# MeryylleA/Lunaris-Orion

Measured on AMD Instinct MI355X. Metric: 128x128 sprites/sec, VAE training step (train_hybrid.py _process_batch), latent_dim=512, higher is better.
Workload: dtype f16; 1 GPU; VAE-only training step (fwd+MSE/KL+bwd+clip+AdamW), per-GPU batch 64, latent_dim 512, teacher scalar 0 (--reward_scale 0 --quality_weight 0; the full hybrid step of BASELINE config 3 is the config3_full_hybrid object of a --full run at N=1), gradient_accumulation_steps 1, fp16 MFMA operands / fp32 accumulate, fp32 master weights; global_batch=64, latent_dim=512, parallelism=single, linear_weight_gradients=factored (never materialised)

## Files before the change

lunaris_orion_amd/csrc/lo_edge.hip:

```cpp
#include "lo_common.h"
#include <stdlib.h>

#define FC_W 128
#define FC_OW 64
#define FC_CO 64

__device__ __forceinline__ void fc_stage_rows(const float* __restrict__ x, float (*xs)[3][FC_W + 2], int n, int oy, int tid) {
  for (int i = tid; i < 3 * 3 * (FC_W + 2); i += 256) {
    int col = i % (FC_W + 2);
    int r = (i / (FC_W + 2)) % 3;
    int ci = i / (3 * (FC_W + 2));
    int iy = 2 * oy - 1 + r, ix = col - 1;
    float v = 0.f;
    if ((unsigned)iy < 128u && (unsigned)ix < 128u) v = x[(((size_t)n * 3 + ci) * 128 + iy) * 128 + ix];
    xs[ci][r][col] = v;
  }
}

template <int ROWS>
__global__ __launch_bounds__(256) void lo_first_conv_fwd_mfma_kernel(const float* __restrict__ x, const float* __restrict__ w,
                                                                     const float* __restrict__ bias, f16* __restrict__ v,
                                                                     float* __restrict__ gn_partial) {
  constexpr int NR = 2 * ROWS + 1, RP = FC_W + 2;
  __shared__ float xs[3][NR][RP];
  __shared__ float ws[FC_CO * 27];
  __shared__ __attribute__((aligned(16))) unsigned char so[FC_OW * 144];
  __shared__ float red[4][8][2];
  const int tid = threadIdx.x, lane = tid & 63, wave = tid >> 6, m = lane & 15, g = lane >> 4;
  const int oy0 = blockIdx.x * ROWS, n = blockIdx.y;
  for (int i = tid; i < 3 * NR * RP; i += 256) {
    const int col = i % RP, r = (i / RP) % NR, ci = i / (RP * NR);
    const int iy = 2 * oy0 - 1 + r, ix = col - 1;
    float val = 0.f;
    if ((unsigned)iy < 128u && (unsigned)ix < 128u) val = x[(((size_t)n * 3 + ci) * 128 + iy) * 128 + ix];
    xs[ci][r][col] = val;
  }
  for (int i = tid; i < FC_CO * 27; i += 256) ws[i] = w[i];
  __syncthreads();
  f16x8 wh[4], wl[4];
#pragma unroll
  for (int mf = 0; mf < 4; ++mf)
#pragma unroll
    for (int j = 0; j < 8; ++j) {
      const int k = 8 * g + j;
      const float wv = k < 27 ? ws[(16 * mf + m) * 27 + k] : 0.f;
      const f16 hi = (f16)wv;
      wh[mf][j] = hi;
      wl[mf][j] = (f16)(wv - (float)hi);
    }
  int koff[8];
#pragma unroll
  for (int j = 0; j < 8; ++j) {
    const int k = 8 * g + j, kk = k < 27 ? k : 0;
    const int ci = kk / 9, r = (kk % 9) / 3, sx = kk % 3;
    koff[j] = (ci * NR + r) * RP + sx;
  }
  f32x4 bv[4];
#pragma unroll
  for (int mf = 0; mf < 4; ++mf) bv[mf] = *reinterpret_cast<const f32x4*>(bias + 16 * mf + 4 * g);
  const float* xbase = &xs[0][0][0];
  const int px = 16 * wave + m;
#pragma unroll 1
  for (int rr = 0; rr < ROWS; ++rr) {
    f16x8 xh, xl;
#pragma unroll
    for (int j = 0; j < 8; ++j) {
      float xv = xbase[koff[j] + 2 * rr * RP + 2 * px];
      if (8 * g + j >= 27) xv = 0.f;
      const f16 hi = (f16)xv;
      xh[j] = hi;
      xl[j] = (f16)(xv - (float)hi);
    }
    float gs[4], gq[4];
#pragma unroll
    for (int mf = 0; mf < 4; ++mf) {
      f32x4 acc = bv[mf];
      acc = __builtin_amdgcn_mfma_f32_16x16x32_f16(wh[mf], xh, acc, 0, 0, 0);
      acc = __builtin_amdgcn_mfma_f32_16x16x32_f16(wl[mf], xh, acc, 0, 0, 0);
      acc = __builtin_amdgcn_mfma_f32_16x16x32_f16(wh[mf], xl, acc, 0, 0, 0);
      const f16x4 h = {(f16)acc[0], (f16)acc[1], (f16)acc[2], (f16)acc[3]};
      *reinterpret_cast<f16x4*>(so + px * 144 + (16 * mf + 4 * g) * 2) = h;
      float s_ = 0.f, q_ = 0.f;
#pragma unroll
      for (int j = 0; j < 4; ++j) { const float a = (float)h[j]; s_ += a; q_ += a * a; }
      gs[mf] = s_; gq[mf] = q_;
    }
#pragma unroll
    for (int mf = 0; mf < 4; ++mf) {
#pragma unroll
      for (int o = 1; o < 32; o <<= 1) { gs[mf] += __shfl_xor(gs[mf], o, 64); gq[mf] += __shfl_xor(gq[mf], o, 64); }
    }
    if (m == 0 && (g & 1) == 0) {
#pragma unroll
      for (int mf = 0; mf < 4; ++mf) { red[wave][2 * mf + (g >> 1)][0] = gs[mf]; red[wave][2 * mf + (g >> 1)][1] = gq[mf]; }
    }
    __syncthreads();
    const int oy = oy0 + rr;
    {
      f16* dst = v + (((size_t)n * 64 + oy) * 64) * FC_CO;
#pragma unroll
      for (int i = 0; i < 2; ++i) {
        const int c = tid + 256 * i, p = c >> 3, ch = c & 7;
        *reinterpret_cast<u32x4*>(dst + p * FC_CO + ch * 8) = *reinterpret_cast<const u32x4*>(so + p * 144 + ch * 16);
      }
    }
    if (tid < 16) {
      const int grp = tid >> 1, which = tid & 1;
      gn_partial[(((size_t)n * 64 + oy) * 8 + grp) * 2 + which] = red[0][grp][which] + red[1][grp][which] + red[2][grp][which] + red[3][grp][which];
    }
    __syncthreads();
  }
}

template <int ROWS>
__global__ __launch_bounds__(256) void lo_first_conv_wgrad_mfma_kernel(const float* __restrict__ x, const f16* __restrict__ dv,
                                                                       float* __restrict__ partial) {
  __shared__ float xs[3][3][FC_W + 2];
  __shared__ __attribute__((aligned(16))) f16 ds[64][FC_CO];
  __shared__ __attribute__((aligned(16))) f16 xt[2][32][64 + 8];
  const int tid = threadIdx.x, n = blockIdx.y, rb = blockIdx.x;
  const int lane = tid & 63, wave = tid >> 6, i16 = lane & 15, q = lane >> 4;
  f32x4 acc[4];
#pragma unroll
  for (int t = 0; t < 4; ++t) acc[t] = (f32x4){0.f, 0.f, 0.f, 0.f};
  constexpr int XN = (3 * 3 * (FC_W + 2) + 255) / 256;
  f16x8 pd[2];
  float px[XN];
  auto prefetch = [&](int oy) __attribute__((always_inline)) {
    const f16* src = dv + (((size_t)n * 64 + oy) * 64) * FC_CO;
#pragma unroll
    for (int j = 0; j < 2; ++j) pd[j] = reinterpret_cast<const f16x8*>(src)[tid + 256 * j];
#pragma unroll
    for (int j = 0; j < XN; ++j) {
      const int i = tid + 256 * j;
      const int col = i % (FC_W + 2), r = (i / (FC_W + 2)) % 3, ci = i / (3 * (FC_W + 2));
      const int iy = 2 * oy - 1 + r, ix = col - 1;
      float v = 0.f;
      if (i < 3 * 3 * (FC_W + 2) && (unsigned)iy < 128u && (unsigned)ix < 128u) v = x[(((size_t)n * 3 + ci) * 128 + iy) * 128 + ix];
      px[j] = v;
    }
  };
  prefetch(rb * ROWS);
  for (int oy = rb * ROWS; oy < rb * ROWS + ROWS; ++oy) {
    __syncthreads();
#pragma unroll
    for (int j = 0; j < 2; ++j) reinterpret_cast<f16x8*>(&ds[0][0])[tid + 256 * j] = pd[j];
#pragma unroll
    for (int j = 0; j < XN; ++j) {
      const int i = tid + 256 * j;
      if (i < 3 * 3 * (FC_W + 2)) (&xs[0][0][0])[i] = px[j];
    }
    if (oy + 1 < rb * ROWS + ROWS) prefetch(oy + 1);
    __syncthreads();
    for (int i = tid; i < 32 * 64; i += 256) {
      const int k = i >> 6, p = i & 63;
      float v = 0.f;
      if (k < 27) {
        const int ci = k / 9, r = (k % 9) / 3, sx = k % 3;
        v = xs[ci][r][2 * p + sx];
      }
      const f16 hi = (f16)v;
      xt[0][k][p] = hi;
      xt[1][k][p] = (f16)(v - (float)hi);
    }
    __syncthreads();
#pragma unroll
    for (int ks = 0; ks < 2; ++ks) {
      const unsigned char* dbase = reinterpret_cast<const unsigned char*>(&ds[0][0]) + (size_t)(32 * ks + 4 * q + (i16 >> 2)) * 128 + wave * 32 + (i16 & 3) * 8;
      h16x4 a_lo = __builtin_amdgcn_ds_read_tr16_b64_v4f16((h16x4 __attribute__((address_space(3)))*)(dbase));
      h16x4 a_hi = __builtin_amdgcn_ds_read_tr16_b64_v4f16((h16x4 __attribute__((address_space(3)))*)(dbase + 16 * 128));
      const f16x8 af = {(f16)a_lo[0], (f16)a_lo[1], (f16)a_lo[2], (f16)a_lo[3], (f16)a_hi[0], (f16)a_hi[1], (f16)a_hi[2], (f16)a_hi[3]};
#pragma unroll
      for (int t = 0; t < 4; ++t) {
        const f16* xr = &xt[t >> 1][16 * (t & 1) + i16][32 * ks + 4 * q];
// ... 32 lines not shown
    for (; k < nrow; k += 16) t += partial[(size_t)k * stride + j];
  }
  red[r][c] = t;
  __syncthreads();
  if (r == 0 && j < ncol) {
    float tot = 0.f;
#pragma unroll
    for (int q = 0; q < 16; ++q) tot += red[q][c];
    out[j] = tot * scale;
  }
}

#define LC_T 16
#define LC_TP (LC_T + 2)
#define LC_CI 32
#define LC_PITCH 80

__device__ __forceinline__ void lc_stage_a4_wide(const f16* __restrict__ a4, unsigned char* tile, int n, int ty, int tx, int tid) {
  constexpr int NCH = LC_TP * LC_TP * 4, NIT = (NCH + 255) / 256;
  u32x4 v[NIT];
#pragma unroll
  for (int k = 0; k < NIT; ++k) {
    const int i = tid + k * 256;
    const int ch = i & 3, p = i >> 2;
    const int y = p / LC_TP, xx = p % LC_TP;
    const int iy = ty * LC_T - 1 + y, ix = tx * LC_T - 1 + xx;
    v[k] = (u32x4){0u, 0u, 0u, 0u};
    if (i < NCH && (unsigned)iy < 128u && (unsigned)ix < 128u)
      v[k] = *reinterpret_cast<const u32x4*>(a4 + (((size_t)n * 128 + iy) * 128 + ix) * LC_CI + ch * 8);
  }
#pragma unroll
  for (int k = 0; k < NIT; ++k) {
    const int i = tid + k * 256;
    if (i < NCH) *reinterpret_cast<u32x4*>(tile + (i >> 2) * LC_PITCH + (i & 3) * 16) = v[k];
  }
}

__device__ __forceinline__ float lc_tanh(float x) { return 1.f - 2.f * __frcp_rn(__expf(2.f * x) + 1.f); }

__global__ __launch_bounds__(256) void lo_final_conv_fwd_mfma_kernel(const f16* __restrict__ a4, const float* __restrict__ w,
                                                                     const float* __restrict__ bias, const float* __restrict__ target,
                                                                     float* __restrict__ recon, float* __restrict__ mse_partial) {
  __shared__ __attribute__((aligned(16))) unsigned char tile[LC_TP * LC_TP * LC_PITCH];
  __shared__ __attribute__((aligned(16))) f16 wf[9 * 4 * 6 * 8];
  __shared__ float red[4];
  const int tid = threadIdx.x, tx = blockIdx.x, ty = blockIdx.y, n = blockIdx.z;
  const int lane = tid & 63, wave = tid >> 6, m = lane & 15, g = lane >> 4;
  lc_stage_a4_wide(a4, tile, n, ty, tx, tid);
  for (int i = tid; i < 3 * LC_CI * 9; i += 256) {
    const int t = i % 9, ci = (i / 9) % LC_CI, co = i / (9 * LC_CI);
    const float wv = w[i];
    const f16 hi = (f16)wv;
    const int slot = ((t * 4 + (ci >> 3)) * 6 + co) * 8 + (ci & 7);
    wf[slot] = hi;
    wf[slot + 24] = (f16)(wv - (float)hi);
  }
  const float bv = m < 3 ? bias[m] : 0.f;
  __syncthreads();
  f16x8 wb[9];
#pragma unroll
  for (int t = 0; t < 9; ++t) {
    wb[t] = (f16x8){0, 0, 0, 0, 0, 0, 0, 0};
    if (m < 6) wb[t] = *reinterpret_cast<const f16x8*>(&wf[((t * 4 + g) * 6 + m) * 8]);
  }
  float sq = 0.f;
#pragma unroll
  for (int rr = 0; rr < 4; ++rr) {
    const int py = wave * 4 + rr;
    f32x4 acc = {0.f, 0.f, 0.f, 0.f};
#pragma unroll
    for (int t = 0; t < 9; ++t) {
      const int r = t / 3, sx = t % 3;
      const f16x8 af = *reinterpret_cast<const f16x8*>(tile + ((py + r) * LC_TP + m + sx) * LC_PITCH + g * 16);
      acc = __builtin_amdgcn_mfma_f32_16x16x32_f16(af, wb[t], acc, 0, 0, 0);
    }
    f32x4 lo;
#pragma unroll
    for (int j = 0; j < 4; ++j) lo[j] = __shfl_down(acc[j], 3, 64);
    if (m < 3) {
      const int oy = ty * LC_T + py, ox = tx * LC_T + 4 * g;
      const size_t o = (((size_t)n * 3 + m) * 128 + oy) * 128 + ox;
      f32x4 rv;
#pragma unroll
      for (int j = 0; j < 4; ++j) rv[j] = lc_tanh(acc[j] + lo[j] + bv);
      *reinterpret_cast<f32x4*>(recon + o) = rv;
      if (mse_partial) {
        const f32x4 tv = *reinterpret_cast<const f32x4*>(target + o);
#pragma unroll
        for (int j = 0; j < 4; ++j) { const float d = rv[j] - tv[j]; sq += d * d; }
      }
    }
  }
  if (mse_partial) {
    const float e = lo_wave_sum(sq);
    if (lane == 0) red[wave] = e;
    __syncthreads();
    if (tid == 0) mse_partial[((size_t)n * gridDim.y + ty) * gridDim.x + tx] = red[0] + red[1] + red[2] + red[3];
  }
}

struct LcBwdArgs {
  const f16* a4;
  const float* w;
  const float* recon;
  const float* target;
  const float* drecon;
  const float* coef;
  float gscale;
  f16* da4;
  float* partial;
};

__device__ __attribute__((aligned(256))) unsigned int lo_zero_page_e[64];
static_assert(sizeof(lo_zero_page_e) >= 1 * 16, "lc_dma_a4: 16 B per lane, all lanes at offset 0 of the zero page");
static_assert(sizeof(lo_zero_page_e) >= 64 * 4, "lc_dma_rt: 64 lanes x 4 B, lane-linear in the zero page");
#define LC_PATCH_BYTES (21 * 1024)
__device__ __forceinline__ void lc_dma_a4(const f16* __restrict__ a4, unsigned int lds_base, int n, int ty, int tx, int wave, int lane) {
  const unsigned char* zpage = reinterpret_cast<const unsigned char*>(lo_zero_page_e);
#pragma unroll
  for (int i = 0; i < 6; ++i) {
    const int k = wave + 4 * i;
    if (k >= 21) break;
    const int q = k * 64 + lane, p = q >> 2, slot = q & 3;
    const int y = p / LC_TP, xx = p - y * LC_TP;
    const int iy = ty * LC_T - 1 + y, ix = tx * LC_T - 1 + xx;
    const void* src = zpage;
    if (p < LC_TP * LC_TP && (unsigned)iy < 128u && (unsigned)ix < 128u) src = a4 + (((size_t)n * 128 + iy) * 128 + ix) * LC_CI + slot * 8;
    lo_dma16(src, __builtin_amdgcn_readfirstlane(lds_base + k * 1024));
  }
}
__device__ __forceinline__ void lo_dma4(const void* gptr, unsigned int lds_off) {
  asm volatile("s_mov_b32 m0, %1\n\ts_nop 0\n\tglobal_load_lds_dword %0, off" ::"v"(gptr), "s"(lds_off) : "memory");
}
__device__ __forceinline__ void lc_dma_rt(const float* __restrict__ recon, const float* __restrict__ gsrc, unsigned int lds_base, int n,
                                          int ty, int tx, int wave, int lane) {
  const unsigned char* zpage = reinterpret_cast<const unsigned char*>(lo_zero_page_e);
#pragma unroll
  for (int jb = 0; jb < 2; ++jb) {
    const int j = wave + 4 * jb;
    if (j * 64 >= LC_TP * LC_TP) break;
    const int p = j * 64 + lane;
    const int y = p / LC_TP, xx = p - y * LC_TP;
    const int iy = ty * LC_T - 1 + y, ix = tx * LC_T - 1 + xx;
    const bool in = p < LC_TP * LC_TP && (unsigned)iy < 128u && (unsigned)ix < 128u;
    const size_t o = ((size_t)n * 3 * 128 + iy) * 128 + ix;
#pragma unroll
    for (int c = 0; c < 3; ++c) {
      lo_dma4(in ? (const void*)(recon + o + c * 16384) : (const void*)(zpage + lane * 4), __builtin_amdgcn_readfirstlane(lds_base + ((0 * 3 + c) * 384 + j * 64) * 4));
// ... 149 lines not shown
  LoProfScope _p("lo_first_conv_wgrad(+sum)", 2.0 * B * 4096 * 64 * 27, (double)B * (3 * 16384 * 4 + 4096 * 64 * 2), st);
  hipLaunchKernelGGL((lo_first_conv_wgrad_mfma_kernel<4>), dim3(16, B), dim3(256), 0, st, x, dv, partial);
  LO_LAUNCH_CHECK("first_conv_wgrad");
  hipLaunchKernelGGL(lo_colsum_kernel, dim3((1728 + 15) / 16), dim3(256), 0, st, partial, dw, B * 16, 1728, 1728, scale);
  LO_LAUNCH_CHECK("first_conv_wgrad_sum");
  return LO_OK;
}
int lo_colsum(const float* partial, float* out, int nrow, int ncol, int stride, float scale, hipStream_t st) {
  hipLaunchKernelGGL(lo_colsum_kernel, dim3((ncol + 15) / 16), dim3(256), 0, st, partial, out, nrow, ncol, stride, scale);
  LO_LAUNCH_CHECK("colsum");
  return LO_OK;
}
int lo_final_conv_fwd(const f16* a4, const float* w, const float* bias, const float* target, float* recon,
                      float* mse_partial, int B, hipStream_t st) {
  LoProfScope _p("lo_final_conv_fwd", 2.0 * B * 16384 * 3 * 288, (double)B * 16384 * (32 * 2 + 3 * 4 * 2), st);
  hipLaunchKernelGGL(lo_final_conv_fwd_mfma_kernel, dim3(8, 8, B), dim3(256), 0, st, a4, w, bias, target, recon, mse_partial);
  LO_LAUNCH_CHECK("final_conv_fwd");
  return LO_OK;
}
int lo_final_conv_bwd(const f16* a4, const float* w, const float* recon, const float* target, const float* drecon,
                      const float* coef, float gscale, f16* da4, float* partial, float* dw, float* db, int B, float scale,
                      hipStream_t st, hipStream_t sum_st, hipEvent_t sum_after) {
  LcBwdArgs a{a4, w, recon, target, drecon, coef, gscale, da4, partial};
  LoProfScope _p("lo_final_conv_bwd(+sums)", 4.0 * B * 16384 * 3 * 288, (double)B * 16384 * (32 * 2 * 2 + 3 * 4 * 2), st);
  constexpr int rows = 8;
  LO_LAUNCH_STOP(lo_final_conv_bwd_kernel<8>, dim3(rows, B), dim3(256), 0, st, a);
  LO_LAUNCH_CHECK("final_conv_bwd");
  if (sum_st && sum_after) { LO_HIP(hipStreamWaitEvent(sum_st, sum_after, 0)); st = sum_st; }
  hipLaunchKernelGGL(lo_colsum_kernel, dim3((864 + 15) / 16), dim3(256), 0, st, partial, dw, B * rows, 864, 867, scale);
  LO_LAUNCH_CHECK("final_conv_dw");
  hipLaunchKernelGGL(lo_colsum_kernel, dim3(1), dim3(256), 0, st, partial + 864, db, B * rows, 3, 867, scale);
// ... 4 lines not shown
```

lunaris_orion_amd/csrc/lo_norm.h:

```cpp
#pragma once
#include "lo_common.h"

int lo_gn_nchunk(int HW, int C);
bool lo_gn_bwd_local_applies(int HW, int C);

struct LoGnLayer { const f16* v; const float* stats; const float* gamma; const float* beta; int B, HW, C; };

struct LoGnFwd {
  const float* partial = nullptr; int MT = 0;
  const float* slab = nullptr; int nsplit = 0; const float* bias = nullptr;
  const f16* other = nullptr;
  int mode = 0;
  f16* y = nullptr;
  uint8_t* y8 = nullptr;
};
int lo_gn_forward(const LoGnLayer& l, const LoGnFwd& op, hipStream_t st);

struct LoGnBwd {
  const f16* dy = nullptr;
  const float* slab = nullptr; int nsplit = 0; const f16* add_src = nullptr; f16* dy_out = nullptr;
  const f16* other = nullptr;
  int mode = 0;
  f16* ds = nullptr;
  f16* dv = nullptr;
// ... 6 lines not shown
enum LoGnBwdForm {
  LO_GNB_SLAB_LOCAL,
  LO_GNB_APPLY_ONLY,
  LO_GNB_LOCAL,
  LO_GNB_TWO_PASS
};
struct LoGnUse { bool slab = false; int rows_in_P1 = 0; bool allow_local = false; };
static inline LoGnUse lo_gn_use(const LoGnBwd& op) { return {op.slab != nullptr, op.rows_in_P1, op.allow_local}; }
struct LoGnChoice { LoGnBwdForm form; LoGnRows rows; };
LoGnChoice lo_gn_bwd_choose(int HW, int C, const LoGnUse& use);
int lo_gn_backward(const LoGnLayer& l, const LoGnBwd& op, hipStream_t st, LoGnRows* rows = nullptr);
int lo_gn_bwd(const LoGnLayer& l, const LoGnBwd& op, float* dgamma, float* dbeta, float* dbias, float scale, hipStream_t st);

struct LoGnFinJob { const float* P1; const float* P2; float* dgamma; float* dbeta; float* dbias; int nblk1, nblk2, C, block0; };
#define LO_GN_FIN_MAX 16
struct LoGnFinJobs { LoGnFinJob j[LO_GN_FIN_MAX]; int n; };
int lo_gn_finalize_all(const LoGnFinJobs& jobs, float scale, hipStream_t st);

int lo_nhwc_to_nchw_f16(const f16* src, f16* dst, int B, int HW, int C, hipStream_t st);
int lo_nchw_to_nhwc_f16(const f16* src, f16* dst, int B, int HW, int C, hipStream_t st, uint8_t* dst8 = nullptr);
int lo_nhwc_f16_to_nchw_f32(const f16* src, float* dst, int B, int HW, int C, float scale, hipStream_t st);
int lo_nchw_f32_to_nhwc_f16(const float* src, f16* dst, int B, int HW, int C, float scale, hipStream_t st);
```

lunaris_orion_amd/csrc/lo_norm.hip:

```cpp
#include "lo_norm.h"
#include <stdlib.h>
#include <type_traits>

#define GN_EPS 1e-5f

enum { GN_MODE_PLAIN = 0, GN_MODE_SKIP = 1, GN_MODE_RES = 2 };

int lo_gn_nchunk(int HW, int C) {
  constexpr long chunk_elems = 16384;
  const long ce = (long)HW * C >= 524288 ? 2 * chunk_elems : chunk_elems;
  long e = (long)HW * C / ce;
  if (e < 1) e = 1;
  if (e > 256) e = 256;
  while (HW % e) --e;
  return (int)e;
}

struct GnFwdArgs {
  const f16* v;
  const float* partial;
  const float* gamma;
  const float* beta;
  const f16* other;
  f16* y;
// ... 418 lines not shown
      g2 += p[1];
      b += P2[(size_t)k * C + c];
    }
  red[0][r][cl] = g1; red[1][r][cl] = g2; red[2][r][cl] = b;
  __syncthreads();
  if (r < 3 && c < C) {
    float tot = 0.f;
#pragma unroll
    for (int q = 0; q < 16; ++q) tot += red[r][q][cl];
    tot *= scale;
    if (r == 0) dbeta[c] = tot; else if (r == 1) dgamma[c] = tot; else dbias[c] = tot;
  }
}

__global__ __launch_bounds__(256) void lo_gn_finalize_all_kernel(LoGnFinJobs jobs, float scale) {
  __shared__ float red[3][64][5];
  int jb = 0;
  while (jb + 1 < jobs.n && (int)blockIdx.x >= jobs.j[jb + 1].block0) ++jb;
  const LoGnFinJob& J = jobs.j[jb];
  const int C = J.C;
  const int cl = threadIdx.x & 3, r = threadIdx.x >> 2;
  const int c = ((int)blockIdx.x - J.block0) * 4 + cl;
  float g1 = 0.f, g2 = 0.f, b = 0.f;
  if (c < C) {
    for (int k = r; k < J.nblk1; k += 64) {
      f32x2 p = *reinterpret_cast<const f32x2*>(J.P1 + ((size_t)k * C + c) * 2);
      g1 += p[0];
      g2 += p[1];
    }
    for (int k = r; k < J.nblk2; k += 64) b += J.P2[(size_t)k * C + c];
  }
  red[0][r][cl] = g1; red[1][r][cl] = g2; red[2][r][cl] = b;
  __syncthreads();
  if (threadIdx.x < 12) {
    const int which = threadIdx.x >> 2, c2 = threadIdx.x & 3;
    const int cg = ((int)blockIdx.x - J.block0) * 4 + c2;
    if (cg < C) {
      float tot = 0.f;
      for (int q = 0; q < 64; ++q) tot += red[which][q][c2];
      tot *= scale;
      if (which == 0) J.dbeta[cg] = tot; else if (which == 1) J.dgamma[cg] = tot; else J.dbias[cg] = tot;
    }
  }
}

__global__ __launch_bounds__(256) void lo_transpose_tile_kernel(const f16* __restrict__ src, f16* __restrict__ dst, uint8_t* __restrict__ dst8,
                                                                int R, int Cc) {
  __shared__ f16 tile[64][66];
  const int n = blockIdx.z, r0 = blockIdx.y * 64, c0 = blockIdx.x * 64;
  const f16* s = src + (size_t)n * R * Cc;
  const int tc = (threadIdx.x & 7) * 8, tr = threadIdx.x >> 3;
#pragma unroll
  for (int p = 0; p < 2; ++p) {
    const int r = tr + 32 * p;
    const f16x8 v = *reinterpret_cast<const f16x8*>(s + (size_t)(r0 + r) * Cc + c0 + tc);
// ... 209 lines not shown
}

int lo_gn_bwd(const LoGnLayer& l, const LoGnBwd& op, float* dgamma, float* dbeta, float* dbias, float scale, hipStream_t st) {
  LoGnRows rows;
  int r = lo_gn_backward(l, op, st, &rows);
  if (r != LO_OK) return r;
  LoProfScope _p3("lo_gn_param_finalize", 0, 0, st);
  hipLaunchKernelGGL(lo_gn_param_finalize_kernel, dim3((l.C + 15) / 16), dim3(256), 0, st, op.P1, op.P2, dgamma, dbeta, dbias,
                     l.B * rows.p1, l.C, scale);
  LO_LAUNCH_CHECK("gn_param_finalize");
  return LO_OK;
}

int lo_gn_finalize_all(const LoGnFinJobs& jobs, float scale, hipStream_t st) {
  int nblocks = 0;
  for (int i = 0; i < jobs.n; ++i) nblocks += (jobs.j[i].C + 3) / 4;
  LoProfScope _p("lo_gn_finalize_all", 0, 0, st);
  hipLaunchKernelGGL(lo_gn_finalize_all_kernel, dim3(nblocks), dim3(256), 0, st, jobs, scale);
  LO_LAUNCH_CHECK("gn_finalize_all");
  return LO_OK;
}

int lo_nhwc_to_nchw_f16(const f16* src, f16* dst, int B, int HW, int C, hipStream_t st) {
  LO_REQUIRE(HW % 64 == 0 && C % 64 == 0, "lo_nhwc_to_nchw_f16: HW=%d, C=%d must be multiples of 64", HW, C);
  LoProfScope _p("lo_layout_transpose", 0, 4.0 * B * HW * C, st);
  LO_LAUNCH_STOP(lo_transpose_tile_kernel, dim3(C / 64, HW / 64, B), dim3(256), 0, st, src, dst, (uint8_t*)nullptr, HW, C);
  LO_LAUNCH_CHECK("nhwc_to_nchw");
  return LO_OK;
}
int lo_nchw_to_nhwc_f16(const f16* src, f16* dst, int B, int HW, int C, hipStream_t st, uint8_t* dst8) {
  LO_REQUIRE(HW % 64 == 0 && C % 64 == 0, "lo_nchw_to_nhwc_f16: HW=%d, C=%d must be multiples of 64", HW, C);
// ... 32 lines not shown
```

lunaris_orion_amd/csrc/lo_vae_step.hip:

```cpp
#include "lo_vae.h"

static int vae_ensure_sync_init(LoVae* h, void* ws, hipStream_t st) {
  if (h->sync_for_ws == ws) return LO_OK;
  hipError_t e = hipSuccess;
  for_each_layer(h, [&](ConvLayer& c) {
    if (e == hipSuccess) e = hipMemsetAsync(WSP(void, c.o_xcnt), 0, (size_t)h->B * 4, st);
    if (e == hipSuccess) e = hipMemsetAsync(WSP(void, c.o_bcnt), 0, (size_t)h->B * 8 * 4, st);
    c.gnf_epoch = 0; c.gba_epoch = 0;
  });
  LO_HIP(e);
  LO_HIP(hipMemsetAsync(WSP(void, h->o_sync_fail), 0, 256, st));
  h->sync_for_ws = ws;
  return LO_OK;
}

static int conv_gn(LoVae* h, ConvLayer& c, const f16* in, const f16* other, f16* y, int mode, const float* P, void* ws,
                   hipStream_t st, size_t o_in8 = 0, size_t o_y8 = 0) {
  LoProfTag tag("fwd kind%d %dx%d %d->%d", c.kind, c.Ho, c.Wo, c.gf.Cin, c.gf.Cout);
  if (c.sk_fwd && !c.f8 && !o_y8) {
    LO_TRY(lo_conv_run(c.gf, {.in = in, .w = WSP(f16, c.o_wp_f), .slab = WSP(float, h->o_skslab), .nsplit = c.sk_fwd}, st));
    tag.end();
    return lo_gn_forward(vae_gn_layer(h, c, P, ws),
                         {.slab = WSP(float, h->o_skslab), .nsplit = c.sk_fwd, .bias = PRM(c.p_b), .other = other, .mode = mode, .y = y}, st);
  }
// ... 147 lines not shown
}

static int vae_gn_finalize(LoVae* h, unsigned enc_mask, bool dec, float* G, void* ws, float inv, hipStream_t st) {
  const int B = h->B;
  LoGnFinJobs jobs;
  jobs.n = 0;
  int blocks = 0;
  bool rows_ok = true;
  auto add = [&](ConvLayer& c) {
    LoGnFinJob& j = jobs.j[jobs.n++];
    j.P1 = WSP(float, c.o_P1); j.P2 = WSP(float, c.o_P2);
    j.dgamma = GRD(c.p_gw); j.dbeta = GRD(c.p_gb); j.dbias = GRD(c.p_b);
    rows_ok = rows_ok && c.np1 > 0 && c.np2 > 0;
    j.nblk1 = B * c.np1; j.nblk2 = B * c.np2;
    j.C = c.Cout; j.block0 = blocks;
    blocks += (c.Cout + 3) / 4;
  };
  for (int s = 0; s < 4; ++s)
    if (enc_mask & (1u << s)) for (int k = 0; k < 3; ++k) add(h->enc[s][k]);
  if (dec) for (int s = 0; s < 4; ++s) add(h->dec[s]);
  LO_REQUIRE(rows_ok, "GroupNorm finalize: a layer's backward has not run (no P1 / P2 rows recorded)");
  return lo_gn_finalize_all(jobs, inv, st);
}

struct LoGapTable { unsigned long long off[80]; int len[80]; int n; };
__global__ void lo_zero_gaps_kernel(float* G, LoGapTable t) {
  const int i = blockIdx.x;
  if (i < t.n && (int)threadIdx.x < t.len[i]) G[t.off[i] + threadIdx.x] = 0.f;
}
static int vae_zero_gaps(LoVae* h, float* G, hipStream_t st) {
  LoGapTable t;
// ... 211 lines not shown
    else
      LO_TRY(gn_backward(c0, {.dy = Gc, .dv = Gd}));
    LO_TRY(lo_first_conv_wgrad(x, dv0, WSP(float, h->o_fcw_part), GRD(c0.p_w), B, inv, st));
    if (dx) LO_TRY(lo_image_dgrad(dv0, 64, 2, PRM(c0.p_w), B, inv, dx, st));
  }
  return LO_OK;
}

int VaeBackward::publish_range(unsigned enc_mask, bool dec) {
  LO_TRY(finalize(enc_mask, dec, h->side));
  LO_HIP(hipEventRecord(h->ev_range, h->side));
  h->range_pending = true;
  return LO_OK;
}

int vae_backward_checks(const LoVae* h, bool args_ok, bool fwd_ran, int fused, const float* target, float loss_scale) {
  LO_REQUIRE(args_ok, "lo_vae_backward: null argument");
  if (!fwd_ran) { lo_set_error("lo_vae_backward: the forward this backward belongs to has not run"); return LO_ERR_STATE; }
  if (fused && (!h->loss_done || !target)) { lo_set_error("lo_vae_backward: fused mode needs lo_vae_loss and a target"); return LO_ERR_STATE; }
  LO_REQUIRE(loss_scale > 0.f, "lo_vae_backward: loss_scale must be positive");
  return LO_OK;
}
}

extern "C" int lo_vae_backward_dx(LoVae* h, const float* x, const float* P, void* ws, const float* recon, const float* target,
                                  int fused, const float* drecon, const float* gmu, const float* glv, float loss_scale,
                                  float* G, float* dx, void* stream) {
  const bool args_ok = h && P && ws && G && x && recon;
  LO_TRY(vae_backward_checks(h, args_ok, args_ok && h->forward_done, fused, target, loss_scale));
  VaeBackward b(h, P, G, ws, loss_scale, stream);
  LO_TRY(b.begin(true));
  const bool fac1 = vae_single_leaves_factors(h) && fused;
  if (fac1 && !h->norm_scratch) { lo_set_error("lo_vae_backward: the factored Linear-gradient mode needs lo_vae_set_gradnorm_scratch"); return LO_ERR_STATE; }
  h->fac.ready = false;
  const bool early = h->norm_scratch && (b.side || fac1);
  LO_TRY(vae_zero_gaps(h, G, (b.side && fused) ? h->side : b.st));
  LO_TRY(b.decoder_chain(fused, recon, target, drecon, fac1, nullptr));
  LO_TRY(b.latent_and_heads(fused, gmu, glv, fac1, true, h->norm_scratch != nullptr));
  if (early) LO_TRY(b.early_norm(fac1));
  LO_TRY(b.encoder_stages(3, 0, x, dx));
  LO_TRY(b.finalize(0xFu, !early, b.st));
  return b.join();
}
extern "C" int lo_vae_backward(LoVae* h, const float* x, const float* P, void* ws, const float* recon, const float* target,
                               int fused, const float* drecon, const float* gmu, const float* glv, float loss_scale,
                               float* G, void* stream) {
  return lo_vae_backward_dx(h, x, P, ws, recon, target, fused, drecon, gmu, glv, loss_scale, G, nullptr, stream);
}

extern "C" int lo_vae_backward_phase(LoVae* h, int phase, const float* x, const float* P, void* ws, const float* recon,
                                     const float* target, int fused, const float* drecon, const float* gmu, const float* glv,
                                     float loss_scale, float* G, void* stream) {
  LO_REQUIRE(phase >= 1 && phase <= 4, "lo_vae_backward_phase: phase must be 1 (final conv, decoder, Linear layers), 2 (whole encoder), "
             "3 (encoder stage 4) or 4 (encoder stages 3..1, after 3)");
  const bool args_ok = h && P && ws && G && x && recon;
  LO_TRY(vae_backward_checks(h, args_ok, args_ok && h->forward_done, fused, target, loss_scale));
  VaeBackward b(h, P, G, ws, loss_scale, stream);
  LO_TRY(b.begin(phase == 1));
  const bool async = b.side && h->async_handover;
  if (phase == 1) {
    const bool facdp = vae_phased_leaves_factors(h) && fused;
    h->fac.ready = false;
    LO_TRY(vae_zero_gaps(h, G, (b.side && fused) ? h->side : b.st));
    LO_TRY(b.decoder_chain(fused, recon, target, drecon, facdp, nullptr));
    LO_TRY(b.latent_and_heads(fused, gmu, glv, facdp, true, async));
    if (facdp) h->fac.scale = b.inv;
    if (async) return b.publish_range(0u, true);
    LO_TRY(b.join());
    return b.finalize(0u, true, b.st);
  }
  LO_TRY(b.encoder_stages(phase == 4 ? 2 : 3, phase == 3 ? 3 : 0, x, nullptr));
  if (phase == 3 && async) {
    LO_TRY(vae_order(h->side, b.st, h->ev_pre));
    return b.publish_range(0x8u, false);
  }
  LO_TRY(b.finalize(phase == 3 ? 0x8u : (phase == 4 ? 0x7u : 0xFu), false, b.st));
  return b.join();
}

// ... 43 lines not shown
```

Baseline: 24660 sprites/s.

## Vectorise first-conv staging, DMA-pipeline final conv fwd, widen GN finalize, reorder zero-gap launch

The first-conv forward and wgrad kernels now stage input rows with float4 loads into a padded LDS layout (zero page for the top halo) and double-buffer the output tile so one barrier per row is dropped. The final-conv forward kernel is templated to process eight tiles per block, using global_load_lds DMA to prefetch the next a4 patch and the target into alternating LDS buffers while computing the current tile. The GN finalize kernel handles 8 channels per block with vectorised, unrolled loads and a shuffle reduction instead of a 64-way LDS loop. The gradient zero-gap clearing is issued on the side stream after the decoder chain is enqueued rather than before. This trades extra code complexity, a larger LDS footprint, fewer blocks in the final conv, and new alignment and evenness requirements for fewer scalar loads and barriers.

```diff
diff --git a/lunaris_orion_amd/csrc/lo_edge.hip b/lunaris_orion_amd/csrc/lo_edge.hip
--- a/lunaris_orion_amd/csrc/lo_edge.hip
+++ b/lunaris_orion_amd/csrc/lo_edge.hip
@@ -1,41 +1,59 @@
 #include "lo_common.h"
 #include <stdlib.h>
+
+__device__ __attribute__((aligned(256))) unsigned int lo_zero_page_e[64];
 
 #define FC_W 128
 #define FC_OW 64
 #define FC_CO 64
 
-__device__ __forceinline__ void fc_stage_rows(const float* __restrict__ x, float (*xs)[3][FC_W + 2], int n, int oy, int tid) {
-  for (int i = tid; i < 3 * 3 * (FC_W + 2); i += 256) {
-    int col = i % (FC_W + 2);
-    int r = (i / (FC_W + 2)) % 3;
-    int ci = i / (3 * (FC_W + 2));
-    int iy = 2 * oy - 1 + r, ix = col - 1;
-    float v = 0.f;
-    if ((unsigned)iy < 128u && (unsigned)ix < 128u) v = x[(((size_t)n * 3 + ci) * 128 + iy) * 128 + ix];
-    xs[ci][r][col] = v;
-  }
+#define FC_X0 4
+#define FC_RP (FC_X0 + FC_W)
+template <int NR, int NIT>
+__device__ __forceinline__ void fc_load_rows(const float* __restrict__ x, f32x4 (&q)[NIT], int n, int iy0, int tid) {
+#pragma unroll
+  for (int k = 0; k < NIT; ++k) {
+    const int i = min(tid + 256 * k, 3 * NR * 32 - 1);
+    const int j = i & 31, row = i >> 5, r = row % NR, ci = row / NR;
+    const int iy = iy0 + r;
+    const float* src = iy >= 0 ? x + (((size_t)n * 3 + ci) * 128 + iy) * 128 + 4 * j : reinterpret_cast<const float*>(lo_zero_page_e);
+    q[k] = *reinterpret_cast<const f32x4*>(src);
+  }
+}
+template <int NR, int NIT>
+__device__ __forceinline__ void fc_store_rows(float* xs, const f32x4 (&q)[NIT], int tid) {
+#pragma unroll
+  for (int k = 0; k < NIT; ++k) {
+    const int i = tid + 256 * k;
+    if (i < 3 * NR * 32) *reinterpret_cast<f32x4*>(xs + (i >> 5) * FC_RP + FC_X0 + 4 * (i & 31)) = q[k];
+  }
+  if (tid < 3 * NR) xs[tid * FC_RP + FC_X0 - 1] = 0.f;
 }
 
 template <int ROWS>
 __global__ __launch_bounds__(256) void lo_first_conv_fwd_mfma_kernel(const float* __restrict__ x, const float* __restrict__ w,
                                                                      const float* __restrict__ bias, f16* __restrict__ v,
                                                                      float* __restrict__ gn_partial) {
-  constexpr int NR = 2 * ROWS + 1, RP = FC_W + 2;
-  __shared__ float xs[3][NR][RP];
-  __shared__ float ws[FC_CO * 27];
-  __shared__ __attribute__((aligned(16))) unsigned char so[FC_OW * 144];
-  __shared__ float red[4][8][2];
+  constexpr int NR = 2 * ROWS + 1, RP = FC_RP, NIT = (3 * NR * 32 + 255) / 256;
+  static_assert(FC_CO * 27 == 432 * 4 && 432 <= 512, "weights: two float4 per thread");
+  __shared__ __attribute__((aligned(16))) float xs[3 * NR * RP];
+  __shared__ __attribute__((aligned(16))) float ws[FC_CO * 27];
+  __shared__ __attribute__((aligned(16))) unsigned char so[2][FC_OW * 144];
+  __shared__ float red[2][4][8][2];
   const int tid = threadIdx.x, lane = tid & 63, wave = tid >> 6, m = lane & 15, g = lane >> 4;
   const int oy0 = blockIdx.x * ROWS, n = blockIdx.y;
-  for (int i = tid; i < 3 * NR * RP; i += 256) {
-    const int col = i % RP, r = (i / RP) % NR, ci = i / (RP * NR);
-    const int iy = 2 * oy0 - 1 + r, ix = col - 1;
-    float val = 0.f;
-    if ((unsigned)iy < 128u && (unsigned)ix < 128u) val = x[(((size_t)n * 3 + ci) * 128 + iy) * 128 + ix];
-    xs[ci][r][col] = val;
-  }
-  for (int i = tid; i < FC_CO * 27; i += 256) ws[i] = w[i];
+  {
+    f32x4 q[NIT], wq[2];
+    fc_load_rows<NR, NIT>(x, q, n, 2 * oy0 - 1, tid);
+#pragma unroll
+    for (int k = 0; k < 2; ++k) wq[k] = reinterpret_cast<const f32x4*>(w)[min(tid + 256 * k, 431)];
+    fc_store_rows<NR, NIT>(xs, q, tid);
+    reinterpret_cast<f32x4*>(ws)[tid] = wq[0];
+    if (tid + 256 < 432) reinterpret_cast<f32x4*>(ws)[tid + 256] = wq[1];
+  }
+  f32x4 bv[4];
+#pragma unroll
+  for (int mf = 0; mf < 4; ++mf) bv[mf] = *reinterpret_cast<const f32x4*>(bias + 16 * mf + 4 * g);
   __syncthreads();
   f16x8 wh[4], wl[4];
 #pragma unroll
@@ -53,19 +71,16 @@
   for (int j = 0; j < 8; ++j) {
     const int k = 8 * g + j, kk = k < 27 ? k : 0;
     const int ci = kk / 9, r = (kk % 9) / 3, sx = kk % 3;
-    koff[j] = (ci * NR + r) * RP + sx;
-  }
-  f32x4 bv[4];
-#pragma unroll
-  for (int mf = 0; mf < 4; ++mf) bv[mf] = *reinterpret_cast<const f32x4*>(bias + 16 * mf + 4 * g);
-  const float* xbase = &xs[0][0][0];
+    koff[j] = (ci * NR + r) * RP + FC_X0 - 1 + sx;
+  }
   const int px = 16 * wave + m;
 #pragma unroll 1
   for (int rr = 0; rr < ROWS; ++rr) {
+    const int cur = rr & 1;
     f16x8 xh, xl;
 #pragma unroll
     for (int j = 0; j < 8; ++j) {
-      float xv = xbase[koff[j] + 2 * rr * RP + 2 * px];
+      float xv = xs[koff[j] + 2 * rr * RP + 2 * px];
       if (8 * g + j >= 27) xv = 0.f;
       const f16 hi = (f16)xv;
       xh[j] = hi;
@@ -79,7 +94,7 @@
       acc = __builtin_amdgcn_mfma_f32_16x16x32_f16(wl[mf], xh, acc, 0, 0, 0);
       acc = __builtin_amdgcn_mfma_f32_16x16x32_f16(wh[mf], xl, acc, 0, 0, 0);
       const f16x4 h = {(f16)acc[0], (f16)acc[1], (f16)acc[2], (f16)acc[3]};
-      *reinterpret_cast<f16x4*>(so + px * 144 + (16 * mf + 4 * g) * 2) = h;
+      *reinterpret_cast<f16x4*>(&so[cur][0] + px * 144 + (16 * mf + 4 * g) * 2) = h;
       float s_ = 0.f, q_ = 0.f;
 #pragma unroll
       for (int j = 0; j < 4; ++j) { const float a = (float)h[j]; s_ += a; q_ += a * a; }
@@ -92,7 +107,7 @@
     }
     if (m == 0 && (g & 1) == 0) {
 #pragma unroll
-      for (int mf = 0; mf < 4; ++mf) { red[wave][2 * mf + (g >> 1)][0] = gs[mf]; red[wave][2 * mf + (g >> 1)][1] = gq[mf]; }
+      for (int mf = 0; mf < 4; ++mf) { red[cur][wave][2 * mf + (g >> 1)][0] = gs[mf]; red[cur][wave][2 * mf + (g >> 1)][1] = gq[mf]; }
     }
     __syncthreads();
     const int oy = oy0 + rr;
@@ -101,21 +116,21 @@
 #pragma unroll
       for (int i = 0; i < 2; ++i) {
         const int c = tid + 256 * i, p = c >> 3, ch = c & 7;
-        *reinterpret_cast<u32x4*>(dst + p * FC_CO + ch * 8) = *reinterpret_cast<const u32x4*>(so + p * 144 + ch * 16);
+        *reinterpret_cast<u32x4*>(dst + p * FC_CO + ch * 8) = *reinterpret_cast<const u32x4*>(&so[cur][0] + p * 144 + ch * 16);
       }
     }
     if (tid < 16) {
       const int grp = tid >> 1, which = tid & 1;
-      gn_partial[(((size_t)n * 64 + oy) * 8 + grp) * 2 + which] = red[0][grp][which] + red[1][grp][which] + red[2][grp][which] + red[3][grp][which];
-    }
-    __syncthreads();
+      gn_partial[(((size_t)n * 64 + oy) * 8 + grp) * 2 + which] =
+          red[cur][0][grp][which] + red[cur][1][grp][which] + red[cur][2][grp][which] + red[cur][3][grp][which];
+    }
   }
 }
 
 template <int ROWS>
 __global__ __launch_bounds__(256) void lo_first_conv_wgrad_mfma_kernel(const float* __restrict__ x, const f16* __restrict__ dv,
                                                                        float* __restrict__ partial) {
-  __shared__ float xs[3][3][FC_W + 2];
+  __shared__ __attribute__((aligned(16))) float xs[3 * 3 * FC_RP];
   __shared__ __attribute__((aligned(16))) f16 ds[64][FC_CO];
   __shared__ __attribute__((aligned(16))) f16 xt[2][32][64 + 8];
   const int tid = threadIdx.x, n = blockIdx.y, rb = blockIdx.x;
@@ -123,33 +138,20 @@
   f32x4 acc[4];
 #pragma unroll
   for (int t = 0; t < 4; ++t) acc[t] = (f32x4){0.f, 0.f, 0.f, 0.f};
-  constexpr int XN = (3 * 3 * (FC_W + 2) + 255) / 256;
   f16x8 pd[2];
-  float px[XN];
+  f32x4 px[2];
   auto prefetch = [&](int oy) __attribute__((always_inline)) {
     const f16* src = dv + (((size_t)n * 64 + oy) * 64) * FC_CO;
 #pragma unroll
     for (int j = 0; j < 2; ++j) pd[j] = reinterpret_cast<const f16x8*>(src)[tid + 256 * j];
-#pragma unroll
-    for (int j = 0; j < XN; ++j) {
-      const int i = tid + 256 * j;
-      const int col = i % (FC_W + 2), r = (i / (FC_W + 2)) % 3, ci = i / (3 * (FC_W + 2));
-      const int iy = 2 * oy - 1 + r, ix = col - 1;
-      float v = 0.f;
-      if (i < 3 * 3 * (FC_W + 2) && (unsigned)iy < 128u && (unsigned)ix < 128u) v = x[(((size_t)n * 3 + ci) * 128 + iy) * 128 + ix];
-      px[j] = v;
-    }
+    fc_load_rows<3, 2>(x, px, n, 2 * oy - 1, tid);
   };
   prefetch(rb * ROWS);
   for (int oy = rb * ROWS; oy < rb * ROWS + ROWS; ++oy) {
     __syncthreads();
 #pragma unroll
     for (int j = 0; j < 2; ++j) reinterpret_cast<f16x8*>(&ds[0][0])[tid + 256 * j] = pd[j];
-#pragma unroll
-    for (int j = 0; j < XN; ++j) {
-      const int i = tid + 256 * j;
-      if (i < 3 * 3 * (FC_W + 2)) (&xs[0][0][0])[i] = px[j];
-    }
+    fc_store_rows<3, 2>(xs, px, tid);
     if (oy + 1 < rb * ROWS + ROWS) prefetch(oy + 1);
     __syncthreads();
     for (int i = tid; i < 32 * 64; i += 256) {
@@ -157,7 +159,7 @@
       float v = 0.f;
       if (k < 27) {
         const int ci = k / 9, r = (k % 9) / 3, sx = k % 3;
-        v = xs[ci][r][2 * p + sx];
+        v = xs[(ci * 3 + r) * FC_RP + FC_X0 - 1 + 2 * p + sx];
       }
       const f16 hi = (f16)v;
       xt[0][k][p] = hi;
@@ -220,39 +222,51 @@
 #define LC_T 16
 #define LC_TP (LC_T + 2)
 #define LC_CI 32
-#define LC_PITCH 80
-
-__device__ __forceinline__ void lc_stage_a4_wide(const f16* __restrict__ a4, unsigned char* tile, int n, int ty, int tx, int tid) {
-  constexpr int NCH = LC_TP * LC_TP * 4, NIT = (NCH + 255) / 256;
-  u32x4 v[NIT];
-#pragma unroll
-  for (int k = 0; k < NIT; ++k) {
-    const int i = tid + k * 256;
-    const int ch = i & 3, p = i >> 2;
-    const int y = p / LC_TP, xx = p % LC_TP;
+
+static_assert(sizeof(lo_zero_page_e) >= 1 * 16, "lc_dma_a4: 16 B per lane, all lanes at offset 0 of the zero page");
+static_assert(sizeof(lo_zero_page_e) >= 64 * 4, "lc_dma_rt: 64 lanes x 4 B, lane-linear in the zero page");
+#define LC_PATCH_BYTES (21 * 1024)
+__device__ __forceinline__ void lc_dma_a4(const f16* __restrict__ a4, unsigned int lds_base, int n, int ty, int tx, int wave, int lane) {
+  const unsigned char* zpage = reinterpret_cast<const unsigned char*>(lo_zero_page_e);
+#pragma unroll
+  for (int i = 0; i < 6; ++i) {
+    const int k = wave + 4 * i;
+    if (k >= 21) break;
+    const int q = k * 64 + lane, p = q >> 2, slot = q & 3;
+    const int y = p / LC_TP, xx = p - y * LC_TP;
     const int iy = ty * LC_T - 1 + y, ix = tx * LC_T - 1 + xx;
-    v[k] = (u32x4){0u, 0u, 0u, 0u};
-    if (i < NCH && (unsigned)iy < 128u && (unsigned)ix < 128u)
-      v[k] = *reinterpret_cast<const u32x4*>(a4 + (((size_t)n * 128 + iy) * 128 + ix) * LC_CI + ch * 8);
-  }
-#pragma unroll
-  for (int k = 0; k < NIT; ++k) {
-    const int i = tid + k * 256;
-    if (i < NCH) *reinterpret_cast<u32x4*>(tile + (i >> 2) * LC_PITCH + (i & 3) * 16) = v[k];
-  }
+    const void* src = zpage;
+    if (p < LC_TP * LC_TP && (unsigned)iy < 128u && (unsigned)ix < 128u) src = a4 + (((size_t)n * 128 + iy) * 128 + ix) * LC_CI + slot * 8;
+    lo_dma16(src, __builtin_amdgcn_readfirstlane(lds_base + k * 1024));
+  }
+}
+__device__ __forceinline__ void lo_dma4(const void* gptr, unsigned int lds_off) {
+  asm volatile("s_mov_b32 m0, %1\n\ts_nop 0\n\tglobal_load_lds_dword %0, off" ::"v"(gptr), "s"(lds_off) : "memory");
 }
 
 __device__ __forceinline__ float lc_tanh(float x) { return 1.f - 2.f * __frcp_rn(__expf(2.f * x) + 1.f); }
 
+template <int TPW>
 __global__ __launch_bounds__(256) void lo_final_conv_fwd_mfma_kernel(const f16* __restrict__ a4, const float* __restrict__ w,
                                                                      const float* __restrict__ bias, const float* __restrict__ target,
                                                                      float* __restrict__ recon, float* __restrict__ mse_partial) {
-  __shared__ __attribute__((aligned(16))) unsigned char tile[LC_TP * LC_TP * LC_PITCH];
+  __shared__ __attribute__((aligned(1024))) unsigned char tile[2][LC_PATCH_BYTES];
+  __shared__ __attribute__((aligned(256))) float tg[2][3][LC_T * LC_T];
   __shared__ __attribute__((aligned(16))) f16 wf[9 * 4 * 6 * 8];
-  __shared__ float red[4];
-  const int tid = threadIdx.x, tx = blockIdx.x, ty = blockIdx.y, n = blockIdx.z;
-  const int lane = tid & 63, wave = tid >> 6, m = lane & 15, g = lane >> 4;
-  lc_stage_a4_wide(a4, tile, n, ty, tx, tid);
+  __shared__ float red[TPW][4];
+  constexpr int WPR = 8 / TPW;
+  const int tid = threadIdx.x, lane = tid & 63, ty = blockIdx.x / WPR, tx0 = (blockIdx.x % WPR) * TPW, n = blockIdx.y;
+  const int wave = __builtin_amdgcn_readfirstlane(tid >> 6), m = lane & 15, g = lane >> 4;
+  const bool has_t = mse_partial != nullptr;
+  const unsigned int tile_lds = (unsigned int)(size_t)(&tile[0][0]);
+  const unsigned int tg_lds = (unsigned int)(size_t)(&tg[0][0][0]);
+  auto dma_target = [&](int buf, int tx) {
+    const float* src = target + (((size_t)n * 3) * 128 + ty * LC_T + wave * 4 + (lane >> 4)) * 128 + tx * LC_T + (lane & 15);
+#pragma unroll
+    for (int c = 0; c < 3; ++c) lo_dma4(src + c * 16384, __builtin_amdgcn_readfirstlane(tg_lds + ((buf * 3 + c) * 256 + wave * 64) * 4));
+  };
+  lc_dma_a4(a4, tile_lds, n, ty, tx0, wave, lane);
+  if (has_t) dma_target(0, tx0);
   for (int i = tid; i < 3 * LC_CI * 9; i += 256) {
     const int t = i % 9, ci = (i / 9) % LC_CI, co = i / (9 * LC_CI);
     const float wv = w[i];
@@ -269,39 +283,53 @@
     wb[t] = (f16x8){0, 0, 0, 0, 0, 0, 0, 0};
     if (m < 6) wb[t] = *reinterpret_cast<const f16x8*>(&wf[((t * 4 + g) * 6 + m) * 8]);
   }
-  float sq = 0.f;
-#pragma unroll
-  for (int rr = 0; rr < 4; ++rr) {
-    const int py = wave * 4 + rr;
-    f32x4 acc = {0.f, 0.f, 0.f, 0.f};
-#pragma unroll
-    for (int t = 0; t < 9; ++t) {
-      const int r = t / 3, sx = t % 3;
-      const f16x8 af = *reinterpret_cast<const f16x8*>(tile + ((py + r) * LC_TP + m + sx) * LC_PITCH + g * 16);
-      acc = __builtin_amdgcn_mfma_f32_16x16x32_f16(af, wb[t], acc, 0, 0, 0);
-    }
-    f32x4 lo;
-#pragma unroll
-    for (int j = 0; j < 4; ++j) lo[j] = __shfl_down(acc[j], 3, 64);
-    if (m < 3) {
-      const int oy = ty * LC_T + py, ox = tx * LC_T + 4 * g;
-      const size_t o = (((size_t)n * 3 + m) * 128 + oy) * 128 + ox;
-      f32x4 rv;
-#pragma unroll
-      for (int j = 0; j < 4; ++j) rv[j] = lc_tanh(acc[j] + lo[j] + bv);
-      *reinterpret_cast<f32x4*>(recon + o) = rv;
-      if (mse_partial) {
-        const f32x4 tv = *reinterpret_cast<const f32x4*>(target + o);
-#pragma unroll
-        for (int j = 0; j < 4; ++j) { const float d = rv[j] - tv[j]; sq += d * d; }
-      }
-    }
-  }
-  if (mse_partial) {
-    const float e = lo_wave_sum(sq);
-    if (lane == 0) red[wave] = e;
+  for (int it = 0; it < TPW; ++it) {
+    const int tx = tx0 + it, cur = it & 1;
+    if (it == 0) asm volatile("s_waitcnt vmcnt(0)" ::: "memory");
+    else asm volatile("s_waitcnt vmcnt(4)" ::: "memory");
+    asm volatile("s_waitcnt lgkmcnt(0)" ::: "memory");
+    __builtin_amdgcn_s_barrier();
+    if (it + 1 < TPW) {
+      lc_dma_a4(a4, tile_lds + (cur ^ 1) * LC_PATCH_BYTES, n, ty, tx + 1, wave, lane);
+      if (has_t) dma_target(cur ^ 1, tx + 1);
+    }
+    const unsigned char* tb = &tile[cur][0];
+    float sq = 0.f;
+#pragma unroll
+    for (int rr = 0; rr < 4; ++rr) {
+      const int py = wave * 4 + rr;
+      f32x4 acc = {0.f, 0.f, 0.f, 0.f};
+#pragma unroll
+      for (int t = 0; t < 9; ++t) {
+        const int r = t / 3, sx = t % 3;
+        const f16x8 af = *reinterpret_cast<const f16x8*>(tb + ((py + r) * LC_TP + m + sx) * 64 + g * 16);
+        acc = __builtin_amdgcn_mfma_f32_16x16x32_f16(af, wb[t], acc, 0, 0, 0);
+      }
+      f32x4 lo;
+#pragma unroll
+      for (int j = 0; j < 4; ++j) lo[j] = __shfl_down(acc[j], 3, 64);
+      if (m < 3) {
+        const int oy = ty * LC_T + py, ox = tx * LC_T + 4 * g;
+        const size_t o = (((size_t)n * 3 + m) * 128 + oy) * 128 + ox;
+        f32x4 rv;
+#pragma unroll
+        for (int j = 0; j < 4; ++j) rv[j] = lc_tanh(acc[j] + lo[j] + bv);
+        *reinterpret_cast<f32x4*>(recon + o) = rv;
+        if (has_t) {
+          const f32x4 tv = *reinterpret_cast<const f32x4*>(&tg[cur][m][py * LC_T + 4 * g]);
+#pragma unroll
+          for (int j = 0; j < 4; ++j) { const float d = rv[j] - tv[j]; sq += d * d; }
+        }
+      }
+    }
+    if (has_t) {
+      const float e = lo_wave_sum(sq);
+      if (lane == 0) red[it][wave] = e;
+    }
+  }
+  if (has_t) {
     __syncthreads();
-    if (tid == 0) mse_partial[((size_t)n * gridDim.y + ty) * gridDim.x + tx] = red[0] + red[1] + red[2] + red[3];
+    if (tid < TPW) mse_partial[((size_t)n * 8 + ty) * 8 + tx0 + tid] = red[tid][0] + red[tid][1] + red[tid][2] + red[tid][3];
   }
 }
 
@@ -317,27 +345,6 @@
   float* partial;
 };
 
-__device__ __attribute__((aligned(256))) unsigned int lo_zero_page_e[64];
-static_assert(sizeof(lo_zero_page_e) >= 1 * 16, "lc_dma_a4: 16 B per lane, all lanes at offset 0 of the zero page");
-static_assert(sizeof(lo_zero_page_e) >= 64 * 4, "lc_dma_rt: 64 lanes x 4 B, lane-linear in the zero page");
-#define LC_PATCH_BYTES (21 * 1024)
-__device__ __forceinline__ void lc_dma_a4(const f16* __restrict__ a4, unsigned int lds_base, int n, int ty, int tx, int wave, int lane) {
-  const unsigned char* zpage = reinterpret_cast<const unsigned char*>(lo_zero_page_e);
-#pragma unroll
-  for (int i = 0; i < 6; ++i) {
-    const int k = wave + 4 * i;
-    if (k >= 21) break;
-    const int q = k * 64 + lane, p = q >> 2, slot = q & 3;
-    const int y = p / LC_TP, xx = p - y * LC_TP;
-    const int iy = ty * LC_T - 1 + y, ix = tx * LC_T - 1 + xx;
-    const void* src = zpage;
-    if (p < LC_TP * LC_TP && (unsigned)iy < 128u && (unsigned)ix < 128u) src = a4 + (((size_t)n * 128 + iy) * 128 + ix) * LC_CI + slot * 8;
-    lo_dma16(src, __builtin_amdgcn_readfirstlane(lds_base + k * 1024));
-  }
-}
-__device__ __forceinline__ void lo_dma4(const void* gptr, unsigned int lds_off) {
-  asm volatile("s_mov_b32 m0, %1\n\ts_nop 0\n\tglobal_load_lds_dword %0, off" ::"v"(gptr), "s"(lds_off) : "memory");
-}
 __device__ __forceinline__ void lc_dma_rt(const float* __restrict__ recon, const float* __restrict__ gsrc, unsigned int lds_base, int n,
                                           int ty, int tx, int wave, int lane) {
   const unsigned char* zpage = reinterpret_cast<const unsigned char*>(lo_zero_page_e);
@@ -517,7 +524,9 @@
 int lo_final_conv_fwd(const f16* a4, const float* w, const float* bias, const float* target, float* recon,
                       float* mse_partial, int B, hipStream_t st) {
   LoProfScope _p("lo_final_conv_fwd", 2.0 * B * 16384 * 3 * 288, (double)B * 16384 * (32 * 2 + 3 * 4 * 2), st);
-  hipLaunchKernelGGL(lo_final_conv_fwd_mfma_kernel, dim3(8, 8, B), dim3(256), 0, st, a4, w, bias, target, recon, mse_partial);
+  LO_REQUIRE((target != nullptr) == (mse_partial != nullptr), "lo_final_conv_fwd: target and mse_partial go together");
+  constexpr int TPW = 8;
+  hipLaunchKernelGGL((lo_final_conv_fwd_mfma_kernel<TPW>), dim3(8 * 8 / TPW, B), dim3(256), 0, st, a4, w, bias, target, recon, mse_partial);
   LO_LAUNCH_CHECK("final_conv_fwd");
   return LO_OK;
 }
diff --git a/lunaris_orion_amd/csrc/lo_norm.h b/lunaris_orion_amd/csrc/lo_norm.h
--- a/lunaris_orion_amd/csrc/lo_norm.h
+++ b/lunaris_orion_amd/csrc/lo_norm.h
@@ -44,6 +44,8 @@
 
 struct LoGnFinJob { const float* P1; const float* P2; float* dgamma; float* dbeta; float* dbias; int nblk1, nblk2, C, block0; };
 #define LO_GN_FIN_MAX 16
+#define LO_GN_FIN_CH 8
+static inline int lo_gn_fin_blocks(int C) { return (C + LO_GN_FIN_CH - 1) / LO_GN_FIN_CH; }
 struct LoGnFinJobs { LoGnFinJob j[LO_GN_FIN_MAX]; int n; };
 int lo_gn_finalize_all(const LoGnFinJobs& jobs, float scale, hipStream_t st);
 
diff --git a/lunaris_orion_amd/csrc/lo_norm.hip b/lunaris_orion_amd/csrc/lo_norm.hip
--- a/lunaris_orion_amd/csrc/lo_norm.hip
+++ b/lunaris_orion_amd/csrc/lo_norm.hip
@@ -456,31 +456,60 @@
 }
 
 __global__ __launch_bounds__(256) void lo_gn_finalize_all_kernel(LoGnFinJobs jobs, float scale) {
-  __shared__ float red[3][64][5];
+  __shared__ float red[4][3][LO_GN_FIN_CH];
   int jb = 0;
   while (jb + 1 < jobs.n && (int)blockIdx.x >= jobs.j[jb + 1].block0) ++jb;
   const LoGnFinJob& J = jobs.j[jb];
   const int C = J.C;
   const int cl = threadIdx.x & 3, r = threadIdx.x >> 2;
-  const int c = ((int)blockIdx.x - J.block0) * 4 + cl;
-  float g1 = 0.f, g2 = 0.f, b = 0.f;
+  const int c0 = ((int)blockIdx.x - J.block0) * LO_GN_FIN_CH;
+  const int c = c0 + cl * 2;
+  float s[6] = {0.f, 0.f, 0.f, 0.f, 0.f, 0.f};
   if (c < C) {
-    for (int k = r; k < J.nblk1; k += 64) {
-      f32x2 p = *reinterpret_cast<const f32x2*>(J.P1 + ((size_t)k * C + c) * 2);
-      g1 += p[0];
-      g2 += p[1];
-    }
-    for (int k = r; k < J.nblk2; k += 64) b += J.P2[(size_t)k * C + c];
-  }
-  red[0][r][cl] = g1; red[1][r][cl] = g2; red[2][r][cl] = b;
-  __syncthreads();
-  if (threadIdx.x < 12) {
-    const int which = threadIdx.x >> 2, c2 = threadIdx.x & 3;
-    const int cg = ((int)blockIdx.x - J.block0) * 4 + c2;
+    const float* p1 = J.P1 + (size_t)c * 2;
+    const int n1 = J.nblk1;
+    int k = r;
+    for (; k + 7 * 64 < n1; k += 8 * 64) {
+      f32x4 v[8];
+#pragma unroll
+      for (int u = 0; u < 8; ++u) v[u] = *reinterpret_cast<const f32x4*>(p1 + (size_t)(k + 64 * u) * C * 2);
+#pragma unroll
+      for (int u = 0; u < 8; ++u) { s[0] += v[u][0]; s[1] += v[u][1]; s[2] += v[u][2]; s[3] += v[u][3]; }
+    }
+    for (; k < n1; k += 64) {
+      const f32x4 v = *reinterpret_cast<const f32x4*>(p1 + (size_t)k * C * 2);
+      s[0] += v[0]; s[1] += v[1]; s[2] += v[2]; s[3] += v[3];
+    }
+    const float* p2 = J.P2 + c;
+    const int n2 = J.nblk2;
+    k = r;
+    for (; k + 7 * 64 < n2; k += 8 * 64) {
+      f32x2 v[8];
+#pragma unroll
+      for (int u = 0; u < 8; ++u) v[u] = *reinterpret_cast<const f32x2*>(p2 + (size_t)(k + 64 * u) * C);
+#pragma unroll
+      for (int u = 0; u < 8; ++u) { s[4] += v[u][0]; s[5] += v[u][1]; }
+    }
+    for (; k < n2; k += 64) {
+      const f32x2 v = *reinterpret_cast<const f32x2*>(p2 + (size_t)k * C);
+      s[4] += v[0]; s[5] += v[1];
+    }
+  }
+#pragma unroll
+  for (int o = 4; o < 64; o <<= 1)
+#pragma unroll
+    for (int q = 0; q < 6; ++q) s[q] += __shfl_xor(s[q], o, 64);
+  const int lane = threadIdx.x & 63, wave = threadIdx.x >> 6;
+  if (lane < 4) {
+    red[wave][0][cl * 2] = s[0]; red[wave][1][cl * 2] = s[1]; red[wave][0][cl * 2 + 1] = s[2]; red[wave][1][cl * 2 + 1] = s[3];
+    red[wave][2][cl * 2] = s[4]; red[wave][2][cl * 2 + 1] = s[5];
+  }
+  __syncthreads();
+  if (threadIdx.x < 3 * LO_GN_FIN_CH) {
+    const int which = threadIdx.x / LO_GN_FIN_CH, c2 = threadIdx.x % LO_GN_FIN_CH;
+    const int cg = c0 + c2;
     if (cg < C) {
-      float tot = 0.f;
-      for (int q = 0; q < 64; ++q) tot += red[which][q][c2];
-      tot *= scale;
+      const float tot = (((red[0][which][c2] + red[1][which][c2]) + red[2][which][c2]) + red[3][which][c2]) * scale;
       if (which == 0) J.dbeta[cg] = tot; else if (which == 1) J.dgamma[cg] = tot; else J.dbias[cg] = tot;
     }
   }
@@ -720,7 +749,12 @@
 
 int lo_gn_finalize_all(const LoGnFinJobs& jobs, float scale, hipStream_t st) {
   int nblocks = 0;
-  for (int i = 0; i < jobs.n; ++i) nblocks += (jobs.j[i].C + 3) / 4;
+  for (int i = 0; i < jobs.n; ++i) {
+    const LoGnFinJob& j = jobs.j[i];
+    LO_REQUIRE(j.C % 2 == 0, "lo_gn_finalize_all: job %d has C=%d, the kernel reads channel pairs", i, j.C);
+    LO_REQUIRE(j.block0 == nblocks, "lo_gn_finalize_all: job %d starts at block %d, expected %d", i, j.block0, nblocks);
+    nblocks += lo_gn_fin_blocks(j.C);
+  }
   LoProfScope _p("lo_gn_finalize_all", 0, 0, st);
   hipLaunchKernelGGL(lo_gn_finalize_all_kernel, dim3(nblocks), dim3(256), 0, st, jobs, scale);
   LO_LAUNCH_CHECK("gn_finalize_all");
diff --git a/lunaris_orion_amd/csrc/lo_vae_step.hip b/lunaris_orion_amd/csrc/lo_vae_step.hip
--- a/lunaris_orion_amd/csrc/lo_vae_step.hip
+++ b/lunaris_orion_amd/csrc/lo_vae_step.hip
@@ -185,7 +185,7 @@
     rows_ok = rows_ok && c.np1 > 0 && c.np2 > 0;
     j.nblk1 = B * c.np1; j.nblk2 = B * c.np2;
     j.C = c.Cout; j.block0 = blocks;
-    blocks += (c.Cout + 3) / 4;
+    blocks += lo_gn_fin_blocks(c.Cout);
   };
   for (int s = 0; s < 4; ++s)
     if (enc_mask & (1u << s)) for (int k = 0; k < 3; ++k) add(h->enc[s][k]);
@@ -427,6 +427,14 @@
   return LO_OK;
 }
 
+template <class Chain>
+int vae_zero_gaps_beside(VaeBackward& b, int fused, Chain&& decoder_chain) {
+  const bool beside = b.side && fused;
+  if (!beside) LO_TRY(vae_zero_gaps(b.h, b.G, b.st));
+  LO_TRY(decoder_chain());
+  if (beside) LO_TRY(vae_zero_gaps(b.h, b.G, b.h->side));
+  return LO_OK;
+}
 int vae_backward_checks(const LoVae* h, bool args_ok, bool fwd_ran, int fused, const float* target, float loss_scale) {
   LO_REQUIRE(args_ok, "lo_vae_backward: null argument");
   if (!fwd_ran) { lo_set_error("lo_vae_backward: the forward this backward belongs to has not run"); return LO_ERR_STATE; }
@@ -447,8 +455,7 @@
   if (fac1 && !h->norm_scratch) { lo_set_error("lo_vae_backward: the factored Linear-gradient mode needs lo_vae_set_gradnorm_scratch"); return LO_ERR_STATE; }
   h->fac.ready = false;
   const bool early = h->norm_scratch && (b.side || fac1);
-  LO_TRY(vae_zero_gaps(h, G, (b.side && fused) ? h->side : b.st));
-  LO_TRY(b.decoder_chain(fused, recon, target, drecon, fac1, nullptr));
+  LO_TRY(vae_zero_gaps_beside(b, fused, [&] { return b.decoder_chain(fused, recon, target, drecon, fac1, nullptr); }));
   LO_TRY(b.latent_and_heads(fused, gmu, glv, fac1, true, h->norm_scratch != nullptr));
   if (early) LO_TRY(b.early_norm(fac1));
   LO_TRY(b.encoder_stages(3, 0, x, dx));
@@ -474,8 +481,7 @@
   if (phase == 1) {
     const bool facdp = vae_phased_leaves_factors(h) && fused;
     h->fac.ready = false;
-    LO_TRY(vae_zero_gaps(h, G, (b.side && fused) ? h->side : b.st));
-    LO_TRY(b.decoder_chain(fused, recon, target, drecon, facdp, nullptr));
+    LO_TRY(vae_zero_gaps_beside(b, fused, [&] { return b.decoder_chain(fused, recon, target, drecon, facdp, nullptr); }));
     LO_TRY(b.latent_and_heads(fused, gmu, glv, facdp, true, async));
     if (facdp) h->fac.scale = b.inv;
     if (async) return b.publish_range(0u, true);
```

Measured after the change: 24880 sprites/s, median of 6. No clear change (+0.9%).
